# xbpeng/DeepMimic

Hardware: NVIDIA H100
Metric: env-steps/sec (30 Hz policy steps; humanoid3d_spinkick, 4096 envs/GPU) (higher is better)
Workload: dtype f32

## Files before the change

deepmimic_b200/csrc/kernels/dm_step.cu:

```cuda
#include "dm_model.cuh"
#include <type_traits>

namespace dmk {

namespace {

template <int W>
struct Tl {
    static __device__ __forceinline__ float shfl(float v, int src) { return __shfl_sync(0xffffffffu, v, src, W); }
    static __device__ __forceinline__ int shfli(int v, int src) { return __shfl_sync(0xffffffffu, v, src, W); }
    static __device__ __forceinline__ V3 shfl3(V3 v, int src) { return mk3(shfl(v.x, src), shfl(v.y, src), shfl(v.z, src)); }
    static __device__ __forceinline__ S6 shfl6(S6 v, int src) { return mks(shfl3(v.a, src), shfl3(v.l, src)); }
};
__device__ __forceinline__ void ld12(const float* p, float* o) {
    const float4 a = reinterpret_cast<const float4*>(p)[0], b = reinterpret_cast<const float4*>(p)[1], c_ = reinterpret_cast<const float4*>(p)[2];
    o[0] = a.x; o[1] = a.y; o[2] = a.z; o[3] = a.w; o[4] = b.x; o[5] = b.y; o[6] = b.z; o[7] = b.w; o[8] = c_.x; o[9] = c_.y; o[10] = c_.z; o[11] = c_.w;
}
__device__ __forceinline__ void st12(float* p, const float* o) {
    reinterpret_cast<float4*>(p)[0] = make_float4(o[0], o[1], o[2], o[3]); reinterpret_cast<float4*>(p)[1] = make_float4(o[4], o[5], o[6], o[7]);
    reinterpret_cast<float4*>(p)[2] = make_float4(o[8], o[9], o[10], o[11]);
}
__device__ __forceinline__ float rcp_fast(float x) { float r; asm("rcp.approx.ftz.f32 %0, %1;" : "=f"(r) : "f"(x)); return r; }
__device__ __forceinline__ int wmax(int v) {
#pragma unroll
// ... 14 lines not shown
        t[0 + j] = s[0] * R.m[j] + s[1] * R.m[3 + j] + s[2] * R.m[6 + j];
        t[3 + j] = s[1] * R.m[j] + s[3] * R.m[3 + j] + s[4] * R.m[6 + j];
        t[6 + j] = s[2] * R.m[j] + s[4] * R.m[3 + j] + s[5] * R.m[6 + j];
    }
    o[0] = R.m[0] * t[0] + R.m[3] * t[3] + R.m[6] * t[6];
    o[1] = R.m[0] * t[1] + R.m[3] * t[4] + R.m[6] * t[7];
    o[2] = R.m[0] * t[2] + R.m[3] * t[5] + R.m[6] * t[8];
    o[3] = R.m[1] * t[1] + R.m[4] * t[4] + R.m[7] * t[7];
    o[4] = R.m[1] * t[2] + R.m[4] * t[5] + R.m[7] * t[8];
    o[5] = R.m[2] * t[2] + R.m[5] * t[5] + R.m[8] * t[8];
}
__device__ __forceinline__ float normalize_angle3(float t) {
    float n = fmodf(t, 6.283185307179586f);
    if (n > 3.14159265358979f) n -= 6.283185307179586f;
    else if (n < -3.14159265358979f) n += 6.283185307179586f;
    return n;
}
__device__ __forceinline__ V3 quat_rotvec3(Q4 q) {
    float s = sqrtf(q.x * q.x + q.y * q.y + q.z * q.z);
    if (!(s > 0.000001f)) return mk3(0.f, 0.f, 0.f);
    float th = normalize_angle3(2.0f * atan2f(s, q.w));
    float k = th / s;
    return mk3(q.x * k, q.y * k, q.z * k);
}
__device__ __forceinline__ Q4 quat_integrate3(V3 omega, Q4 quat, bool base_body, float dt) {
    V3 angvel = base_body ? omega : qrot(quat, omega);
    float fAngle = sqrtf(dot(angvel, angvel));
    const float kThr = 0.5f * 1.57079632679489661923f;
    if (fAngle * dt > kThr) fAngle = kThr / dt;
    V3 axis;
    if (fAngle < 0.001f) axis = angvel * (0.5f * dt - (dt * dt * dt) * 0.020833333333f * fAngle * fAngle);
    else axis = angvel * (__sinf(0.5f * fAngle * dt) / fAngle);
    float cw = __cosf(fAngle * dt * 0.5f);
    Q4 r = base_body ? qmul(quat, mkq(-axis.x, -axis.y, -axis.z, cw)) : qmul(mkq(axis.x, axis.y, axis.z, cw), quat);
    float n = rsqrtf(r.x * r.x + r.y * r.y + r.z * r.z + r.w * r.w);
    return mkq(r.x * n, r.y * n, r.z * n, r.w * n);
}

enum LkSlot { kLC = 0 , kLM = 3,
              kLD = 4 , kLThr = 7,
              kLWd = 8 , kLInt = 14 , kLInt2 = 15 ,
              kLWb = 16 , kLFlg = 22 , kLTree = 23 ,
              kLAx = 24 , kLTl = 27,
              kLZr = 28 ,
              kLHe = 32 , kLKp = 35,
              kLKd = 36, kLLo = 37, kLHi = 38, kLChild = 39 ,
              kLDc = 40 , kLMc = 43 ,
              kLDyn = 44 , kLDChild = 45 ,
              kLkFloats = 48 };
__device__ __forceinline__ float4 ld4(const float* p) { return *reinterpret_cast<const float4*>(p); }
enum HdrSlot { kHLayout = 0, kHLvc = 24, kHGrav = 32 , kHh = 35, kHScale = 36, kHMu = 37, kHFdt = 38, kHDmax = 39 , kHdrFloats = 40 };
__device__ __forceinline__ float* step_smem() { extern __shared__ __align__(16) float dm_step_sm[]; return dm_step_sm; }

}

int dm_step_layout(int nl, int n, int chain_len, int maxrows, int W, StepLayout* L) {
    const int maxpts = maxrows / 3;
    int o = 0;
    L->nl = nl; L->n = n; L->chain_len = chain_len; L->maxrows = maxrows; L->maxpts = maxpts;
    L->oU = o; o += nl * 24;
    L->oR = o; o += nl * 12;
    L->oA = o;
    const int world = nl * 24, tri = maxrows * (maxrows + 1) / 2;
    L->oW = o; L->oV = o + nl * 12;
    L->oPp = o + world; L->oQ = L->oPp + maxpts * 4;
    const int pre = world + maxpts * 4 + 4 * 8;
    o += (pre > tri ? pre : tri);
    o = (o + 3) & ~3;
    const int ys = dm_step_y_stride(W), scr = 28 * (nl - 1);
    L->oY = o; o += (chain_len * ys > scr) ? chain_len * ys : scr;
    L->oLam = o; o += maxrows; o += (o & 1); L->oRhs = o; o += maxrows; L->oInv = o; o += maxrows;
    L->oRl = o; o += maxrows;
    L->oPi = o; o += maxpts; L->oPr = o; o += maxpts;
    L->oG = o; o += 21 + 13 + 2;
    L->oZ = o; o += ((n + 3) / 4) * 4;
    L->env_floats = ((o + 15) / 32) * 32 + 16;
    L->hot_floats = kHdrFloats + ((nl * kLkFloats + (nl * nl + nl * chain_len + 3) / 4 + 3) / 4) * 4;
    return L->hot_floats * 4 + 0;
}
int dm_step_smem_bytes(const StepLayout& L, int tiles) { return (L.hot_floats + L.env_floats * tiles) * static_cast<int>(sizeof(float)); }

constexpr int kSubstepBarriers = 2;
constexpr int kPgsBlock = 2;
enum PgsSection { kSecLimit = 0, kSecNormal = 1, kSecFriction = 2 };
template <int W, int S, int ST, int B>
__device__ __forceinline__ void pgs_sweeps(const float* sA, float* sLam, const float2* sRI, int lane, int NL, int P, int NLmax, int Pmax, float mu) {
    using T = Tl<W>;
    float w[S];
#pragma unroll
    for (int s = 0; s < S; ++s) w[s] = 0.f;
    int tjs[S];
#pragma unroll
    for (int s = 0; s < S; ++s) { const int rid = lane + s * W; tjs[s] = rid * (rid + 1) / 2; }
    auto tri = [](int i) { return (i * (i + 1)) >> 1; };
    auto a_own = [&](int s, int i, int ti) -> float {
        if (ST > 0) return sA[i * ST + lane + s * W];
        const int rid = lane + s * W;
        return sA[(rid >= i) ? (tjs[s] + i) : (ti + rid)];
    };
    auto a_pair = [&](int i, int j, int ti, int tj_) -> float {
        if (ST > 0) return sA[i * ST + j];
        return sA[(i >= j) ? (ti + j) : (tj_ + i)];
    };
#pragma unroll 1
    for (int p = 0; p < Pmax; ++p) {
        const int i = NL + ((p < P) ? p : 0);
        const float l0 = (p < P) ? sLam[i] : 0.f;
#pragma unroll
        for (int s = 0; s < S; ++s) w[s] = fmaf(a_own(s, i, tri(i)), l0, w[s]);
    }
    bool writer[B];
#pragma unroll
    for (int k = 0; k < B; ++k) writer[k] = lane == k;
    auto block = [&](int pos0, int it, auto sec_tag) {
        constexpr int SEC = decltype(sec_tag)::value;
        int ik[B], tk[B]; bool vk[B];
        float tot = 0.f;
        float wk[B], rhs[B], inv[B], lam[B], lo[B], hi[B], ain[B * (B - 1) / 2 > 0 ? B * (B - 1) / 2 : 1], ao[S][B];
        if (SEC == kSecLimit) {
#pragma unroll
            for (int k = 0; k < B; ++k) { const int pos = pos0 + k; vk[k] = pos < NL; ik[k] = vk[k] ? ((it & 1) ? pos : NL - 1 - pos) : 0; }
        } else {
            const int i0 = ((SEC == kSecNormal) ? NL : NL + P) + pos0, cnt = (SEC == kSecNormal) ? P : 2 * P;
#pragma unroll
            for (int k = 0; k < B; ++k) { ik[k] = i0 + k; vk[k] = pos0 + k < cnt; }
        }
#pragma unroll
        for (int k = 0; k < B; ++k) tk[k] = (ST > 0) ? 0 : tri(ik[k]);
// ... 133 lines not shown
                        f.a.x -= ti * ub.z; f.a.y -= ti * ub.w; f.a.z -= ti * uc.x; f.l.x -= ti * uc.y; f.l.y -= ti * uc.z; f.l.z -= ti * uc.w;
                    }
                }
                if (nd >= 1) {
                    float t = qa.x * f.a.x + qa.y * f.a.y + qa.z * f.a.z;
                    if (first && kind == 0) { t = lsign; rvel = lsign * sQ[24 + rid]; }
                    const float y = t * uf.y;
                    if (rv_) sY[dp0 * YS + rid] = y;
                    acc += y * y;
                    const float ti = t * ue.z;
                    f.a.x -= ti * ua.x; f.a.y -= ti * ua.y; f.a.z -= ti * ua.z; f.l.x -= ti * ua.w; f.l.y -= ti * ub.x; f.l.z -= ti * ub.y;
                }
                first = false;
                f = shift_f(f, mk3(qc.y, qc.z, qc.w));
                if (par < 0) break;
                cur = par;
            }
            {
                float x[6] = {f.a.x, f.a.y, f.a.z, f.l.x, f.l.y, f.l.z};
                int o = 0;
#pragma unroll
                for (int i = 0; i < 6; ++i) {
#pragma unroll
                    for (int k = 0; k < i; ++k) x[i] -= sG[o++] * x[k];
                    x[i] *= sG[15 + i];
                    if (rv_) sY[i * YS + rid] = x[i];
                    acc += x[i] * x[i];
                }
            }
            if (rv_) {
                const float inv = acc > 1.1920929e-7f ? 1.0f / acc : 0.f;
                float rhs, lam0 = 0.f;
                if (kind == 1) {
                    float perr = 0.f, verr = -rvel;
                    if (pdist > 0.f) verr -= pdist / h; else perr = -pdist * 0.2f / h;
                    rhs = perr * inv + verr * inv;
                    lam0 = sPi[p] * 0.85f;
                } else if (kind != 0) rhs = -rvel * inv;
                else {
                    float perr = 0.f, verr = -rvel;
                    const bool combine = lpen > -0.04f;
                    if (lpen > 0.f) verr = -lpen / h; else perr = -lpen * 0.2f / h;
                    rhs = combine ? (perr * inv + verr * inv) : (verr * inv);
                }
                sRI[rid] = make_float2(rhs, inv); sLam[rid] = lam0;
            }
        }
    }
    __syncwarp();
    SPROF(7);
    const int Pmax = (W == 32) ? P : wmax(P);
    const int NLmax = (W == 32) ? NL : wmax(NL);
    {
        constexpr int kSq2 = (W == 16) ? 22 : 36;
        const int region = max(nl * 24, MR * (MR + 1) / 2);
        const int mode = (nslots == 1) ? 0 : ((NRmax <= kSq2 && kSq2 * kSq2 + W <= region) ? 1 : 2);
        const int st = (mode == 0) ? W : kSq2;
        auto put = [&](int i, int j, float v) {
            if (mode != 2) { sA[i * st + j] = v; sA[j * st + i] = v; }
            else { const int hi_ = max(i, j), lo_ = min(i, j); sA[hi_ * (hi_ + 1) / 2 + lo_] = v; }
        };
#pragma unroll 1
        for (int j = 0; j < NLmax; ++j) {
            const bool jv = j < NL;
            const int bj = jv ? sRl[j] : 0;
#pragma unroll 1
            for (int i0 = 0; i0 < NRmax; i0 += W) {
                const int i = i0 + lane;
                const bool pv = jv && i < NR && i >= j;
                const int cd = pv ? CD[sRl[i] * nl + bj] : 0;
                const float* yi = sY + (pv ? i : 0); const float* yj = sY + (jv ? j : 0);
                float acc = 0.f;
#pragma unroll 1
                for (int k = 0; k < CL; k += 4, yi += 4 * YS, yj += 4 * YS) {
                    const float a0 = yi[0], a1 = yi[YS], a2 = yi[2 * YS], a3 = yi[3 * YS];
                    const float b0 = yj[0], b1 = yj[YS], b2 = yj[2 * YS], b3 = yj[3 * YS];
                    if (k < cd) acc += a0 * b0;
                    if (k + 1 < cd) acc += a1 * b1;
                    if (k + 2 < cd) acc += a2 * b2;
                    if (k + 3 < cd) acc += a3 * b3;
                }
                if (pv) put(i, j, acc);
            }
        }
        const int npp = P * (P + 1) / 2, nppmax = Pmax * (Pmax + 1) / 2;
#pragma unroll 1
        for (int q0 = 0; q0 < nppmax; q0 += W) {
            const int q = q0 + lane;
            const bool pv = q < npp;
            int pp = static_cast<int>((sqrtf(8.0f * static_cast<float>(q) + 1.0f) - 1.0f) * 0.5f);
            if (pp * (pp + 1) / 2 > q) --pp;
            if ((pp + 1) * (pp + 2) / 2 <= q) ++pp;
            const int pr = q - pp * (pp + 1) / 2;
            const int in_p = pv ? NL + pp : 0, it_p = pv ? NL + P + 2 * pp : 0, in_r = pv ? NL + pr : 0, it_r = pv ? NL + P + 2 * pr : 0;
            const int cd = pv ? CD[sRl[in_p] * nl + sRl[in_r]] : 0;
            const float* ypn = sY + in_p; const float* ypt = sY + it_p; const float* yrn = sY + in_r; const float* yrt = sY + it_r;
            float acc[3][3];
#pragma unroll
            for (int x = 0; x < 3; ++x)
#pragma unroll
                for (int y = 0; y < 3; ++y) acc[x][y] = 0.f;
#pragma unroll 1
            for (int k = 0; k < CL; k += 4, ypn += 4 * YS, ypt += 4 * YS, yrn += 4 * YS, yrt += 4 * YS) {
                float av[3][4], bv[3][4];
#pragma unroll
                for (int d = 0; d < 4; ++d) {
                    av[0][d] = ypn[d * YS]; av[1][d] = ypt[d * YS]; av[2][d] = ypt[d * YS + 1];
                    bv[0][d] = yrn[d * YS]; bv[1][d] = yrt[d * YS]; bv[2][d] = yrt[d * YS + 1];
                }
#pragma unroll
                for (int d = 0; d < 4; ++d)
                    if (k + d < cd) {
#pragma unroll
                        for (int x = 0; x < 3; ++x)
#pragma unroll
                            for (int y = 0; y < 3; ++y) acc[x][y] += av[x][d] * bv[y][d];
                    }
            }
            if (pv) {
                if (mode != 2) {
                    float* rp[3] = {sA + in_p * st, sA + it_p * st, sA + it_p * st + st};
                    float* rr[3] = {sA + in_r * st, sA + it_r * st, sA + it_r * st + st};
                    const int cp[3] = {in_p, it_p, it_p + 1}, cr[3] = {in_r, it_r, it_r + 1};
#pragma unroll
                    for (int x = 0; x < 3; ++x)
#pragma unroll
                        for (int y = 0; y < 3; ++y) { rp[x][cr[y]] = acc[x][y]; rr[y][cp[x]] = acc[x][y]; }
                } else {
#pragma unroll
                    for (int x = 0; x < 3; ++x)
#pragma unroll
                        for (int y = 0; y < 3; ++y) put(x == 0 ? in_p : it_p + x - 1, y == 0 ? in_r : it_r + y - 1, acc[x][y]);
                }
            }
        }
        __syncwarp();
        SPROF(8);
        if (mode == 0) pgs_sweeps<W, 1, W, kPgsBlock>(sA, sLam, sRI, lane, NL, P, NLmax, Pmax, mu);
        else if (mode == 1) pgs_sweeps<W, kSlots, kSq2, kPgsBlock>(sA, sLam, sRI, lane, NL, P, NLmax, Pmax, mu);
        else pgs_sweeps<W, kSlots, 0, kPgsBlock>(sA, sLam, sRI, lane, NL, P, NLmax, Pmax, mu);
    }
    SPROF(9);
#pragma unroll 1
    for (int p = lane; p < P; p += W) {
        if (alive) {
            const int ref = sPr[p];
            float* mpt = mani + (ref >> 2) * kManifoldFloats + (ref & 3) * 12;
            mpt[7] = sLam[NL + p]; mpt[8] = sLam[NL + P + 2 * p]; mpt[9] = sLam[NL + P + 2 * p + 1];
        }
    }
    {
        const int info = (lane < nl) ? lk_i(lane) : 0;
        const int nd = (info >> 16) & 0xff, dp0 = (info >> 24) & 0xff;
        const int d0 = (lane < nl) ? (lk_i2(lane) & 0xff) : 0;
        float z0 = 0.f, z1 = 0.f, z2 = 0.f, zb = 0.f;
        const int kb = (lane < 6) ? lane : 0;
        const bool mine = lane < nl && nd > 0;
        const int need = dp0 + nd - 1;
        const unsigned char* cdl = CD + lane;
#pragma unroll 2
        for (int i = 0; i < NRmax; ++i) {
            const int b = sRl[i];
            const float l = (i < NR) ? sLam[i] : 0.f;
            const float yb = sY[kb * YS + i], y0 = sY[dp0 * YS + i], y1 = sY[(dp0 + 1) * YS + i], y2 = sY[(dp0 + 2) * YS + i];
            const bool in = mine && cdl[b * nl] > need;
            zb = fmaf(yb, l, zb);
            if (in) { z0 = fmaf(y0, l, z0); if (nd == 3) { z1 = fmaf(y1, l, z1); z2 = fmaf(y2, l, z2); } }
        }
        if (lane < 6) sZ[lane] = zb;
        if (lane < nl && nd >= 1) sZ[d0] = z0;
        if (lane < nl && nd == 3) { sZ[d0 + 1] = z1; sZ[d0 + 2] = z2; }
    }
    __syncwarp();
}


struct Ctx {
    float* E;
    const int* LYS;
    const float* LK;
    int lane, li;
    int plane, level, ndof, jtype, maxlevel;
    bool act;
};
__device__ __forceinline__ const StepLayout& lay_of(const Ctx& c) { return *reinterpret_cast<const StepLayout*>(c.LYS); }
template <int W>
__device__ __forceinline__ Ctx make_ctx() {
    Ctx c;
    float* sm = step_smem();
    c.LYS = reinterpret_cast<const int*>(sm + kHLayout); c.LK = sm + kHdrFloats;
    const StepLayout& LY = *reinterpret_cast<const StepLayout*>(c.LYS);
    const int tile = threadIdx.x / W;
    c.lane = threadIdx.x % W;
// ... 23 lines not shown
template <int W>
__device__ __noinline__ void kin_pass(float4 jp, float4 jv) {
    const Ctx c = make_ctx<W>();
    using T = Tl<W>;
    const StepLayout& LY = lay_of(c);
    float* sS = c.E + LY.oR; float* sW = c.E + LY.oW; float* sV = c.E + LY.oV; const float* sB = c.E + LY.oG + 21;
    const float* LKo = c.LK + c.li * kLkFloats;
    const float4 ax4 = ld4(LKo + kLAx), zr4 = ld4(LKo + kLZr), c4 = ld4(LKo + kLC);
    const V3 axis = mk3(ax4.x, ax4.y, ax4.z);
    const Q4 zrot = mkq(zr4.x, zr4.y, zr4.z, zr4.w);
    const V3 cvec = mk3(c4.x, c4.y, c4.z);
    Q4 cached;
    if (c.jtype == kJSpherical) cached = qmul(mkq(jp.x, jp.y, jp.z, -jp.w), zrot);
    else if (c.jtype == kJRevolute) {
        float s, co;
        __sincosf(-0.5f * jp.x, &s, &co);
        cached = qmul(mkq(axis.x * s, axis.y * s, axis.z * s, co), zrot);
    } else cached = zrot;
    const M3 R = qmat(cached);
    V3 jw = mk3(0, 0, 0);
    if (c.jtype == kJSpherical) jw = mk3(jv.x, jv.y, jv.z); else if (c.jtype == kJRevolute) jw = jv.x * axis;
    M3 Rwl; V3 Pw, cw; S6 vel;
    if (c.lane == 0) {
        const M3 Rwb = qmat(mkq(sB[3], sB[4], sB[5], sB[6]));
        const V3 bo = mk3(sB[7], sB[8], sB[9]);
        Rwl = mul(R, Rwb); cw = mulT(Rwb, cvec); Pw = mk3(sB[0], sB[1], sB[2]) + cw;
        vel = mks(bo + mulT(Rwl, jw), mk3(sB[10], sB[11], sB[12]) + cross(bo, cw));
    }
#pragma unroll 1
    for (int lv = 1; lv <= c.maxlevel; ++lv) {
        M3 pR; V3 pp; S6 pv;
#pragma unroll
        for (int k = 0; k < 9; ++k) pR.m[k] = T::shfl(Rwl.m[k], c.plane);
        pp = T::shfl3(Pw, c.plane);
        pv = T::shfl6(vel, c.plane);
        if (c.level == lv) {
            Rwl = mul(R, pR); cw = mulT(pR, cvec); Pw = pp + cw;
            vel = mks(pv.a + mulT(Rwl, jw), pv.l + cross(pv.a, cw));
        }
    }
    if (c.act) {
        const float4 d4 = ld4(LKo + kLD);
        const V3 dw = mulT(Rwl, mk3(d4.x, d4.y, d4.z));
        V3 S0 = mk3(Rwl.m[0], Rwl.m[1], Rwl.m[2]);
        if (c.jtype != kJSpherical) S0 = mulT(Rwl, axis);
        const float wr[12] = {Rwl.m[0], Rwl.m[1], Rwl.m[2], Rwl.m[3], Rwl.m[4], Rwl.m[5], Rwl.m[6], Rwl.m[7], Rwl.m[8], Pw.x, Pw.y, Pw.z};
        const float qr[12] = {S0.x, S0.y, S0.z, Rwl.m[3], Rwl.m[4], Rwl.m[5], Rwl.m[6], Rwl.m[7], Rwl.m[8], cw.x, cw.y, cw.z};
        const float vr[12] = {vel.a.x, vel.a.y, vel.a.z, vel.l.x, vel.l.y, vel.l.z, dw.x, dw.y, dw.z, 0.f, 0.f, 0.f};
        st12(sW + c.lane * 12, wr); st12(sS + c.lane * 12, qr); st12(sV + c.lane * 12, vr);
    }
    __syncwarp();
}

template <int W>
__device__ __noinline__ int collide(float* mani, int alive, int mcnt) {
    const Ctx c = make_ctx<W>();
    const float scale = step_smem()[kHScale];
    using T = Tl<W>;
    const StepLayout& LY = lay_of(c);
    const float* sW = c.E + LY.oW; const float* sV = c.E + LY.oV;
    float* sPp = c.E + LY.oPp; float* sPi = c.E + LY.oPi; int* sPr = reinterpret_cast<int*>(c.E + LY.oPr);
    const float* LKo = c.LK + c.li * kLkFloats;
    const int shape = reinterpret_cast<const int*>(LKo)[kLFlg] & 0xff;
    int cnt = 0;
    float mp[48];
    M3 Rwl;
    float wrec[12], vrec[12];
    ld12(sW + c.li * 12, wrec); ld12(sV + c.li * 12, vrec);
#pragma unroll
    for (int k = 0; k < 9; ++k) Rwl.m[k] = wrec[k];
    const float thr = LKo[kLThr];
    const float4 he4 = ld4(LKo + kLHe);
    const V3 he = mk3(he4.x, he4.y, he4.z);
    const V3 pos = mk3(wrec[9] + vrec[6], wrec[10] + vrec[7], wrec[11] + vrec[8]);
    V3 dl = mul(Rwl, mk3(0.f, -1.f, 0.f));
    V3 vtx;
    if (shape == kSBox) vtx = mk3(dl.x >= 0 ? he.x : -he.x, dl.y >= 0 ? he.y : -he.y, dl.z >= 0 ? he.z : -he.z);
    else {
        V3 sup = mk3(0, 0, 0);
        if (shape == kSCapsule) sup = mk3(0.f, (dl.y >= 0.f) ? he.y : -he.y, 0.f);
        float inv = rsqrtf(dot(dl, dl));
        vtx = sup + (he.x * inv) * dl;
    }
    const V3 vw = pos + mulT(Rwl, vtx);
    const float dist = vw.y;
    const bool need = c.act && alive && (mcnt > 0 || dist < thr);
    {
        const float4* mg = reinterpret_cast<const float4*>(mani + c.li * kManifoldFloats);
#pragma unroll
        for (int k = 0; k < 12; ++k) { float4 v = need ? mg[k] : make_float4(0.f, 0.f, 0.f, 0.f); mp[4 * k] = v.x; mp[4 * k + 1] = v.y; mp[4 * k + 2] = v.z; mp[4 * k + 3] = v.w; }
    }
#pragma unroll
    for (int k = 0; k < 4; ++k) if (mp[k * 12] != 0.f && cnt == k) cnt = k + 1;
    if (c.act && dist < thr) {
        float best = thr * thr; int nearest = -1;
#pragma unroll
        for (int k = 0; k < 4; ++k) if (k < cnt) {
            float dx = mp[k * 12 + 1] - vtx.x, dy = mp[k * 12 + 2] - vtx.y, dz = mp[k * 12 + 3] - vtx.z, dd = dx * dx + dy * dy + dz * dz;
            if (dd < best) { best = dd; nearest = k; }
        }
        int idx = nearest;
        float k7 = 0, k8 = 0, k9 = 0, k11 = 0;
        if (nearest >= 0) {
#pragma unroll
            for (int k = 0; k < 4; ++k) if (k == nearest) { k7 = mp[k * 12 + 7]; k8 = mp[k * 12 + 8]; k9 = mp[k * 12 + 9]; k11 = mp[k * 12 + 11]; }
        } else if (cnt < 4) { idx = cnt; cnt++; }
        else {
            int mpi = -1; float mpen = dist;
#pragma unroll
            for (int k = 0; k < 4; ++k) if (mp[k * 12 + 10] < mpen) { mpi = k; mpen = mp[k * 12 + 10]; }
            auto Pt = [&](int k) { return mk3(mp[k * 12 + 1], mp[k * 12 + 2], mp[k * 12 + 3]); };
            auto area = [&](V3 a, V3 b) { V3 x = cross(a, b); return dot(x, x); };
            float res[4] = {0, 0, 0, 0};
            if (mpi != 0) res[0] = area(vtx - Pt(1), Pt(3) - Pt(2));
            if (mpi != 1) res[1] = area(vtx - Pt(0), Pt(3) - Pt(2));
            if (mpi != 2) res[2] = area(vtx - Pt(0), Pt(3) - Pt(1));
            if (mpi != 3) res[3] = area(vtx - Pt(0), Pt(2) - Pt(1));
            idx = 0; float bv = fabsf(res[0]);
#pragma unroll
            for (int k = 1; k < 4; ++k) if (fabsf(res[k]) > bv) { bv = fabsf(res[k]); idx = k; }
        }
#pragma unroll
        for (int k = 0; k < 4; ++k) if (k == idx) {
            float* q = mp + k * 12;
            q[0] = 1.f; q[1] = vtx.x; q[2] = vtx.y; q[3] = vtx.z; q[4] = vw.x; q[5] = 0.f; q[6] = vw.z; q[7] = k7; q[8] = k8; q[9] = k9; q[10] = dist; q[11] = k11;
        }
    }
#pragma unroll
    for (int k = 3; k >= 0; --k) if (k < cnt) {
        V3 pa = pos + mulT(Rwl, mk3(mp[k * 12 + 1], mp[k * 12 + 2], mp[k * 12 + 3]));
        mp[k * 12 + 10] = pa.y - mp[k * 12 + 5];
        mp[k * 12 + 11] += 1.f;
    }
#pragma unroll
    for (int k = 3; k >= 0; --k) if (k < cnt) {
        V3 pa = pos + mulT(Rwl, mk3(mp[k * 12 + 1], mp[k * 12 + 2], mp[k * 12 + 3]));
        bool rm = !(mp[k * 12 + 10] <= thr);
        if (!rm) {
            float dx = mp[k * 12 + 4] - pa.x, dy = mp[k * 12 + 5] - (pa.y - mp[k * 12 + 10]), dz = mp[k * 12 + 6] - pa.z;
            rm = (dx * dx + dy * dy + dz * dz) > thr * thr;
        }
        if (rm) {
            const int last = cnt - 1;
#pragma unroll
            for (int l2 = 0; l2 < 4; ++l2) if (l2 == last) {
                if (k != l2) for (int j = 0; j < 12; ++j) mp[k * 12 + j] = mp[l2 * 12 + j];
                mp[l2 * 12] = 0.f;
            }
            cnt--;
        }
    }
    if (!c.act || !alive) cnt = 0;
    int tol = 0;
#pragma unroll
    for (int k = 0; k < 4; ++k) if (k < cnt && mp[k * 12 + 10] <= 0.001f * scale) tol = 1;
    if (need) {
        float4* mo = reinterpret_cast<float4*>(mani + c.li * kManifoldFloats);
#pragma unroll
        for (int k = 0; k < 12; ++k) mo[k] = make_float4(mp[4 * k], mp[4 * k + 1], mp[4 * k + 2], mp[4 * k + 3]);
    }
    int incl = cnt, over = 0;
#pragma unroll
    for (int o = 1; o < W; o <<= 1) { int t = __shfl_up_sync(0xffffffffu, incl, o, W); if (c.lane >= o) incl += t; }
    const int base = incl - cnt;
#pragma unroll
    for (int k = 0; k < 4; ++k) if (k < cnt) {
        const int p = base + k;
        if (p < LY.maxpts) {
            V3 pa = pos + mulT(Rwl, mk3(mp[k * 12 + 1], mp[k * 12 + 2], mp[k * 12 + 3]));
            sPp[p * 4] = pa.x; sPp[p * 4 + 1] = pa.y; sPp[p * 4 + 2] = pa.z; sPp[p * 4 + 3] = mp[k * 12 + 10];
            sPi[p] = mp[k * 12 + 7];
            sPr[p] = c.lane * 4 + k;
        } else over = 1;
    }
    const int P = min(T::shfli(incl, W - 1), LY.maxpts);
    __syncwarp();
    return P | (tol << 8) | (over << 9) | (cnt << 10);
}

template <int W>
__device__ __noinline__ float3 aba_solve(float g0, float g1, float g2, float kdt, int bullet, float jvx, float jvy, float jvz) {
    const Ctx c = make_ctx<W>();
    const float gx = step_smem()[kHGrav], gy = step_smem()[kHGrav + 1], gz = step_smem()[kHGrav + 2], h = step_smem()[kHh];
    using T = Tl<W>;
    const StepLayout& LY = lay_of(c);
    float* sU = c.E + LY.oU; const float* sS = c.E + LY.oR; const float* sW = c.E + LY.oW; float* sV = c.E + LY.oV; float* sG = c.E + LY.oG; float* sB = sG + 21;
    const float* LKo = c.LK + c.li * kLkFloats;
    const int dyn = c.act ? reinterpret_cast<const int*>(LKo)[kLDyn] : (100 << 8);
    const int dpar = dyn & 0xff, dlev = static_cast<int>(static_cast<signed char>((dyn >> 8) & 0xff)), byp = (dyn >> 16) & 0xff, dnch = (dyn >> 24) & 0xff;
    const int dchild = reinterpret_cast<const int*>(LKo)[kLDChild];
    const int dmax = reinterpret_cast<const int*>(step_smem())[kHDmax];
    const bool isroot = c.lane == 0;
    const float4 dc4 = ld4(LKo + kLDc);
    const float mass = c.act ? dc4.w : 0.f;
    float q[12];
    ld12(sS + c.li * 12, q);
    const V3 S0 = mk3(q[0], q[1], q[2]), S1 = mk3(q[3], q[4], q[5]), S2 = mk3(q[6], q[7], q[8]), cwk = mk3(q[9], q[10], q[11]);
    V3 cw = cwk;
    if (byp != 0xff) { const float* qb = sS + byp * 12; cw = cw + mk3(qb[9], qb[10], qb[11]); }
    if (isroot) cw = mk3(0, 0, 0);
    float vv[8];
    {
        const float4 a = reinterpret_cast<const float4*>(sV + c.li * 12)[0], b = reinterpret_cast<const float4*>(sV + c.li * 12)[1];
        vv[0] = a.x; vv[1] = a.y; vv[2] = a.z; vv[3] = a.w; vv[4] = b.x; vv[5] = b.y;
    }
    const S6 velk = mks(mk3(vv[0], vv[1], vv[2]), mk3(vv[3], vv[4], vv[5]));
    S6 vel = velk;
    if (isroot) vel = mks(mk3(sB[7], sB[8], sB[9]), mk3(sB[10], sB[11], sB[12]));
    V3 jww = mk3(0, 0, 0);
    if (c.jtype == kJSpherical) jww = jvx * S0 + jvy * S1 + jvz * S2; else if (c.jtype == kJRevolute) jww = jvx * S0;
    S6 ab;
    {
        const S6 cj = mks(cross(vel.a, jww), cross(vel.l, jww));
        if (isroot) {
            const V3 bo = vel.a, bv = vel.l;
            V3 wxv;
            if (bullet) wxv = cross(bo, bv);
            else {
                const M3 Rwb = qmat(mkq(sB[3], sB[4], sB[5], sB[6]));
                wxv = mulT(Rwb, cross(bo, mul(Rwb, bv)));
            }
            ab = mks(mk3(0, 0, 0), mk3(-gx, -gy, -gz) - wxv);
        }
#pragma unroll 1
        for (int lv = 0; lv <= dmax; ++lv) {
            S6 pa = T::shfl6(ab, dpar);
            if (dlev == lv) ab = shift_m(pa, cw) + cj;
        }
    }
    Art IA; S6 pA;
// ... 472 lines not shown
        }
        PROF(1);
        if (stage == total_stages) break;
        if (__syncthreads_and(!alive)) break;
        PROF(2);
        if (__ballot_sync(0xffffffffu, alive) == 0u) {
            if ((stage % stages_per_upd) != 0)
                for (int k = 0; k < kSubstepBarriers; ++k) __syncthreads();
            continue;
        }
        const int ph = stage % stages_per_upd;
        if (ph == 0) {
            int cb = 0;
            if constexpr (TASK) {
                if (__ballot_sync(0xffffffffu, alive && need_action) != 0u) {
                    const V3 com = tile_com<W>(E + LY.oW + li * 12, sV + li * 12, act ? LKo[kLM] : 0.f, 1.0f / (M.total_mass * scale));
                    if (lane == 0 && alive && need_action) { tk[kKPrevCom] = com.x; tk[kKPrevCom + 1] = com.y; tk[kKPrevCom + 2] = com.z; }
                }
            }
            if (lane == 0 && alive) {
                const double timer = tm[kTTimer] + dt;
                double kin_time = tm[kTKin];
                double dur_ = M.motion_dur;
                if constexpr (TASK) dur_ = st.ctab->info[st.clip[env]].dur;
                const double dur = dur_;
                double p0 = kin_time / dur; p0 -= floor(p0);
                kin_time += dt;
                double p1 = kin_time / dur; p1 -= floor(p1);
                if constexpr (TASK) {
                    const ClipInfo& ci = st.ctab->info[st.clip[env]];
                    if (ci.loop && p1 < p0 && M.sync_root_pos) {
                        const double simq[4] = {static_cast<double>(sB[3]), static_cast<double>(sB[4]), static_cast<double>(sB[5]), static_cast<double>(sB[6])};
                        kin_wrap_sync(frame_times + ci.frame_off, frames + static_cast<size_t>(ci.frame_off) * M.pose_dim, M.pose_dim, ci.num_frames, ci.cycle_delta, dur, kin_time,
                                      tm + kTOrigin, tm + kTOriginRot, static_cast<double>(sB[0]) / M.scale, static_cast<double>(sB[2]) / M.scale, simq, true, false);
                    }
                } else if (M.loop_motion && p1 < p0 && (M.sync_root_pos || M.sync_root_rot)) {
                    const double simq[4] = {static_cast<double>(sB[3]), static_cast<double>(sB[4]), static_cast<double>(sB[5]), static_cast<double>(sB[6])};
                    kin_wrap_sync(frame_times, frames, M.pose_dim, M.num_frames, M.cycle_delta, dur, kin_time, tm + kTOrigin, tm + kTOriginRot,
                                  static_cast<double>(sB[0]) / M.scale, static_cast<double>(sB[2]) / M.scale, simq, M.sync_root_pos != 0, M.sync_root_rot != 0);
                }
                const double ctrl_time = tm[kTCtrl] + dt;
                if (need_action) tm[kTPrevAct] = ctrl_time;
                tm[kTTimer] = timer; tm[kTKin] = kin_time; tm[kTCtrl] = ctrl_time;
                {
                    const double cur = ctrl_time + tm[kTInitOff], pad = 0.001 * dt, T_ = M.query_dt;
                    int c0 = static_cast<int>(floor((cur + pad) / T_)), c1 = static_cast<int>(floor((cur + pad - dt) / T_));
                    cb = (c0 != c1) ? 1 : 0;
                }
                if (timer >= tm[kTTimerMax]) cb |= 2;
                if (M.end_at_clip_end && kin_time >= dur) cb |= 4;
            }
            cbits = T::shfli(cb, 0);
            need_action = 0;
            PROF(3);
            const float4 tg = reinterpret_cast<const float4*>(sim + 16 + 8 * nl)[li];
            float e0 = 0, e1 = 0, e2 = 0;
            if (jtype == kJSpherical) {
                Q4 q = mkq(jp.x, jp.y, jp.z, jp.w);
                Q4 dq = qmul(q, mkq(jv.x, jv.y, jv.z, 0.f));
                Q4 qi = qnormalize(mkq(q.x + 0.5f * fdt * dq.x, q.y + 0.5f * fdt * dq.y, q.z + 0.5f * fdt * dq.z, q.w + 0.5f * fdt * dq.w));
                V3 e = quat_rotvec3(qmul(qconj(qi), mkq(tg.x, tg.y, tg.z, tg.w)));
                e0 = e.x; e1 = e.y; e2 = e.z;
            } else if (jtype == kJRevolute) {
                e0 = tg.x - (normalize_angle3(jp.x) + fdt * jv.x);
            }
            const float kp = LKo[kLKp], kd = LKo[kLKd];
            const float pe0 = kp * e0, pe1 = kp * e1, pe2 = kp * e2;
            const float3 qdd = aba_solve<W>(pe0 - kd * jv.x, pe1 - kd * jv.y, pe2 - kd * jv.z, fdt * kd, 0, jv.x, jv.y, jv.z);
            float t0 = 0, t1 = 0, t2 = 0;
            if (ndof >= 1) t0 = pe0 + kd * (-jv.x - fdt * qdd.x);
            if (ndof == 3) { t1 = pe1 + kd * (-jv.y - fdt * qdd.y); t2 = pe2 + kd * (-jv.z - fdt * qdd.z); }
            const float mag = sqrtf(t0 * t0 + t1 * t1 + t2 * t2), tlim = LKo[kLTl];
            if (mag > tlim) { float s = tlim / mag; t0 *= s; t1 *= s; t2 *= s; }
            tau0 = t0; tau1 = t1; tau2 = t2;
            PROF(4);
            continue;
        }
        int P;
        {
            const int r = collide<W>(mani, alive ? 1 : 0, mcnt);
            P = r & 0xff; in_contact_tol = ((r >> 8) & 1) != 0; if ((r >> 9) & 1) f_over = 1; mcnt = (r >> 10) & 7;
        }
        PROF(3);
        {
            const float3 qdd = aba_solve<W>(tau0, tau1, tau2, 0.f, 1, jv.x, jv.y, jv.z);
            bool hit = false;
            if (ndof >= 1) { const float v = jv.x + h * qdd.x; jv.x = cl100(v); hit |= fabsf(v) > 100.f; }
            if (ndof == 3) { const float v1 = jv.y + h * qdd.y, v2 = jv.z + h * qdd.z; jv.y = cl100(v1); jv.z = cl100(v2); hit |= fabsf(v1) > 100.f || fabsf(v2) > 100.f; }
            if (lane == 0) for (int k = 0; k < 6; ++k) hit |= fabsf(sB[7 + k]) >= 100.f;
            const unsigned hb = __ballot_sync(0xffffffffu, hit);
            if (hb != 0u) {
                const unsigned hseg = (W == 32) ? hb : ((hb >> (threadIdx.x & 16)) & 0xffffu);
                vel_pass<W>(jv.x, jv.y, jv.z, hseg != 0u);
            }
        }
        PROF(ph == 1 ? 16 : 17);
        __syncthreads();
        PROF(2);
        int lim_dir = 0; float lim_pen = 0.f;
        if (act && has_limit && alive) {
            float p0 = jp.x - LKo[kLLo], p1 = LKo[kLHi] - jp.x;
            if (!(p0 > 0.f)) { lim_dir = 1; lim_pen = p0; }
            else if (!(p1 > 0.f)) { lim_dir = -1; lim_pen = p1; }
        }
        const unsigned lbal = __ballot_sync(0xffffffffu, lim_dir != 0);
        const unsigned lseg = (W == 32) ? lbal : ((lbal >> (threadIdx.x & 16)) & 0xffffu);
        int NL = __popc(lseg);
        const unsigned anyrow = __ballot_sync(0xffffffffu, NL + P > 0);
        last_nr = 0;
        if (anyrow != 0) {
            {
                const int lidx = __popc(lseg & ((1u << lane) - 1u));
                if (NL > 8) { NL = 8; f_over = 1; }
                if (lim_dir != 0 && lidx < 8) { sQ[lidx] = __int_as_float(lane); sQ[8 + lidx] = (lim_dir == -1) ? -1.f : 1.f; sQ[16 + lidx] = lim_pen; sQ[24 + lidx] = jv.x; }
            }
            if (NL + 3 * P > LY.maxrows) { P = (LY.maxrows - NL) / 3; f_over = 1; }
            const int NR = NL + 3 * P;
            last_nr = NR;
            __syncwarp();
            PROF(5);
#ifdef DM_PROFILE
            { const int nrm = wmax(NR); if ((threadIdx.x & 31) == 0) { PRF[13] += nrm; PRF[14] += 1; if (nrm > W) PRF[15] += 1; } }
#endif
            solve_rows<W>(NL, P, mani, alive ? 1 : 0, PRFP);
            PROF(10);
            const float3 dq = dv_pass<W>();
            if (NR > 0) {
                if (ndof >= 1) jv.x = cl100(jv.x + dq.x);
                if (ndof == 3) { jv.y = cl100(jv.y + dq.y); jv.z = cl100(jv.z + dq.z); }
            }
            PROF(11);
        }
        __syncthreads();
        PROF(2);
        if (lane == 0) {
            sB[0] += h * sB[10]; sB[1] += h * sB[11]; sB[2] += h * sB[12];
            const Q4 q = quat_integrate3(mk3(sB[7], sB[8], sB[9]), mkq(sB[3], sB[4], sB[5], sB[6]), true, h);
            sB[3] = q.x; sB[4] = q.y; sB[5] = q.z; sB[6] = q.w;
        }
        if (jtype == kJRevolute) jp.x += h * jv.x;
        else if (jtype == kJSpherical) { Q4 q = quat_integrate3(mk3(jv.x, jv.y, jv.z), mkq(jp.x, jp.y, jp.z, jp.w), false, h); jp = make_float4(q.x, q.y, q.z, q.w); }
        __syncwarp();
        need_kin = true;
        if (ph == sim_substeps) pending_flags = true;
        PROF(12);
    }
#ifdef DM_PROFILE
    __syncwarp();
    if ((threadIdx.x & 31) == 0 && st.prof) { unsigned int* o = st.prof + (blockIdx.x * (blockDim.x / 32) + threadIdx.x / 32) * kProfCounters; for (int k = 0; k < kProfCounters; ++k) o[k] = PRF[k]; }
#endif
}

const StepKernel kStepKernels[2][2] = {{dm_step_kernel<16, false>, dm_step_kernel<16, true>}, {dm_step_kernel<32, false>, dm_step_kernel<32, true>}};

constexpr int kEnvOrderItems = 4;
__global__ void __launch_bounds__(kEnvOrderThreads) dm_env_order_kernel(const int* __restrict__ load, int n_padded, int tiles, int W, int* __restrict__ order) {
    constexpr int kWarps = kEnvOrderThreads / 32, kCells = kEnvOrderItems * kWarps, kChunk = kEnvOrderItems * kEnvOrderThreads;
    constexpr int kParts = kEnvOrderThreads / kLoadBuckets, kPer = kCells / kParts;
    static_assert(kParts <= 32 && 32 % kParts == 0 && kCells % kParts == 0, "the scan of a bucket's cells runs inside one warp");
    __shared__ int base[kLoadBuckets];
    __shared__ int cnt[kLoadBuckets][kCells + 1];
    const int t = threadIdx.x, warp = t / 32, lane = t % 32;
    const unsigned lt = (1u << lane) - 1u;
    int b[kEnvOrderItems];
    auto load_chunk = [&](int c0) {
#pragma unroll
        for (int i = 0; i < kEnvOrderItems; ++i) { const int e = c0 + i * kEnvOrderThreads + t; b[i] = (e < n_padded) ? env_load_bucket(load[e]) : kLoadBuckets; }
    };
    auto count = [&](int bk) {
        const unsigned peers = __match_any_sync(0xffffffffu, bk);
        if (bk < kLoadBuckets && (peers & lt) == 0) atomicAdd(&base[bk], __popc(peers));
    };
    load_chunk(0);
    if (t < kLoadBuckets) base[t] = 0;
    __syncthreads();
// ... 48 lines not shown
```

Before: 2.513 million.

## Enlarge W=16 square PGS matrix region and alias scratch arrays into it

For 16-wide tiles, the square (non-packed) PGS matrix stride grows from 22 to 24. The layout now reserves at least a 24x24 region, so the square mode is always chosen when the row count fits, rather than falling back to packed triangular indexing. To pay for the larger region, the Pi and Z scratch arrays are aliased into the same region for W=16, which shrinks the per-env footprint elsewhere. This risks lifetime conflicts between the aliased buffers and the matrix, and it changes shared-memory size and therefore occupancy. Profiling counters and a compile-time switch to force packed mode are also added.

After: 2.579 million (median of 6 runs). +2.6%, better.

```diff
diff --git a/deepmimic_b200/csrc/kernels/dm_step.cu b/deepmimic_b200/csrc/kernels/dm_step.cu
--- a/deepmimic_b200/csrc/kernels/dm_step.cu
+++ b/deepmimic_b200/csrc/kernels/dm_step.cu
@@ -90,6 +90,8 @@
 enum HdrSlot { kHLayout = 0, kHLvc = 24, kHGrav = 32 , kHh = 35, kHScale = 36, kHMu = 37, kHFdt = 38, kHDmax = 39 , kHdrFloats = 40 };
 __device__ __forceinline__ float* step_smem() { extern __shared__ __align__(16) float dm_step_sm[]; return dm_step_sm; }
 
+__host__ __device__ constexpr int pgs_sq2(int W) { return W == 16 ? 24 : 36; }
+
 }
 
 int dm_step_layout(int nl, int n, int chain_len, int maxrows, int W, StepLayout* L) {
@@ -102,16 +104,22 @@
     const int world = nl * 24, tri = maxrows * (maxrows + 1) / 2;
     L->oW = o; L->oV = o + nl * 12;
     L->oPp = o + world; L->oQ = L->oPp + maxpts * 4;
-    const int pre = world + maxpts * 4 + 4 * 8;
-    o += (pre > tri ? pre : tri);
+    int pre = world + maxpts * 4 + 4 * 8, region = tri;
+    if (W == 16) {
+        L->oPi = o + pre; pre += maxpts;
+        L->oZ = o;
+        if (pgs_sq2(W) * pgs_sq2(W) > region) region = pgs_sq2(W) * pgs_sq2(W);
+    }
+    o += (pre > region ? pre : region);
     o = (o + 3) & ~3;
     const int ys = dm_step_y_stride(W), scr = 28 * (nl - 1);
     L->oY = o; o += (chain_len * ys > scr) ? chain_len * ys : scr;
     L->oLam = o; o += maxrows; o += (o & 1); L->oRhs = o; o += maxrows; L->oInv = o; o += maxrows;
     L->oRl = o; o += maxrows;
-    L->oPi = o; o += maxpts; L->oPr = o; o += maxpts;
+    if (W != 16) { L->oPi = o; o += maxpts; }
+    L->oPr = o; o += maxpts;
     L->oG = o; o += 21 + 13 + 2;
-    L->oZ = o; o += ((n + 3) / 4) * 4;
+    if (W != 16) { L->oZ = o; o += ((n + 3) / 4) * 4; }
     L->env_floats = ((o + 15) / 32) * 32 + 16;
     L->hot_floats = kHdrFloats + ((nl * kLkFloats + (nl * nl + nl * chain_len + 3) / 4 + 3) / 4) * 4;
     return L->hot_floats * 4 + 0;
@@ -351,9 +359,13 @@
     const int Pmax = (W == 32) ? P : wmax(P);
     const int NLmax = (W == 32) ? NL : wmax(NL);
     {
-        constexpr int kSq2 = (W == 16) ? 22 : 36;
+        constexpr int kSq2 = pgs_sq2(W);
         const int region = max(nl * 24, MR * (MR + 1) / 2);
-        const int mode = (nslots == 1) ? 0 : ((NRmax <= kSq2 && kSq2 * kSq2 + W <= region) ? 1 : 2);
+#ifdef DM_PGS_PACKED
+        const int mode = (nslots == 1) ? 0 : 2;
+#else
+        const int mode = (nslots == 1) ? 0 : ((NRmax <= kSq2 && (W == 16 || kSq2 * kSq2 + W <= region)) ? 1 : 2);
+#endif
         const int st = (mode == 0) ? W : kSq2;
         auto put = [&](int i, int j, float v) {
             if (mode != 2) { sA[i * st + j] = v; sA[j * st + i] = v; }
@@ -438,6 +450,9 @@
         if (mode == 0) pgs_sweeps<W, 1, W, kPgsBlock>(sA, sLam, sRI, lane, NL, P, NLmax, Pmax, mu);
         else if (mode == 1) pgs_sweeps<W, kSlots, kSq2, kPgsBlock>(sA, sLam, sRI, lane, NL, P, NLmax, Pmax, mu);
         else pgs_sweeps<W, kSlots, 0, kPgsBlock>(sA, sLam, sRI, lane, NL, P, NLmax, Pmax, mu);
+#ifdef DM_PROFILE
+        if (mode != 0 && (threadIdx.x & 31) == 0) prf[6] += static_cast<unsigned int>(clock64()) - pt;
+#endif
     }
     SPROF(9);
 #pragma unroll 1
@@ -1337,7 +1352,10 @@
             __syncwarp();
             PROF(5);
 #ifdef DM_PROFILE
-            { const int nrm = wmax(NR); if ((threadIdx.x & 31) == 0) { PRF[13] += nrm; PRF[14] += 1; if (nrm > W) PRF[15] += 1; } }
+            {
+                const int nrm = wmax(NR);
+                if ((threadIdx.x & 31) == 0) { PRF[13] += nrm; PRF[14] += 1; if (nrm > W) PRF[15] += (nrm > pgs_sq2(W)) ? 65536u : 1u; }
+            }
 #endif
             solve_rows<W>(NL, P, mani, alive ? 1 : 0, PRFP);
             PROF(10);
```

## Process contact manifolds with four lanes per link instead of one

Applied to the files above, without the earlier changes.

Contact manifold update in collide is restructured so each link needing collision work is handled by a quad of lanes, one per cached contact point, processed in compacted passes via ballots. This removes the 48-float per-thread manifold array, which is large in registers or local memory, and the serial per-point loops. The cost is extra shuffles, ballots and a pass loop, plus explicit rounding intrinsics to keep results matching. A profiling marker index also changes.

New measurement: 2.531 million before, 2.577 million after, median of 6. 1.8% higher.

```diff
diff --git a/deepmimic_b200/csrc/kernels/dm_step.cu b/deepmimic_b200/csrc/kernels/dm_step.cu
--- a/deepmimic_b200/csrc/kernels/dm_step.cu
+++ b/deepmimic_b200/csrc/kernels/dm_step.cu
@@ -567,6 +567,31 @@
     __syncwarp();
 }
 
+__device__ __forceinline__ V3 link_point(const M3& R, V3 pos, V3 p) {
+    return mk3(__fadd_rn(pos.x, __fmaf_rn(R.m[6], p.z, __fmaf_rn(R.m[0], p.x, __fmul_rn(R.m[3], p.y)))),
+               __fadd_rn(pos.y, __fmaf_rn(R.m[7], p.z, __fmaf_rn(R.m[1], p.x, __fmul_rn(R.m[4], p.y)))),
+               __fadd_rn(pos.z, __fmaf_rn(R.m[8], p.z, __fmaf_rn(R.m[2], p.x, __fmul_rn(R.m[5], p.y)))));
+}
+
+template <int W>
+__device__ __forceinline__ int sort_cached_points(V3 own, float own_dist, V3 p, float dist) {
+    const int s = threadIdx.x & 3, q0 = (threadIdx.x % W) & ~3;
+    auto qshfl = [&](float x, int k) { return Tl<W>::shfl(x, q0 + k); };
+    int mpi = -1; float mpen = dist;
+#pragma unroll
+    for (int k = 0; k < 4; ++k) { const float pen = qshfl(own_dist, k); if (pen < mpen) { mpi = k; mpen = pen; } }
+    auto pt = [&](int k) { return mk3(qshfl(own.x, k), qshfl(own.y, k), qshfl(own.z, k)); };
+    const V3 pa = pt(s == 0 ? 1 : 0), pb = pt(s == 3 ? 2 : 3), pc = pt(s <= 1 ? 2 : 1);
+    const float ax = p.x - pa.x, ay = p.y - pa.y, az = p.z - pa.z;
+    const float bx = pb.x - pc.x, by = pb.y - pc.y, bz = pb.z - pc.z;
+    const float cx = __fmaf_rn(ay, bz, -__fmul_rn(az, by)), cy = __fmaf_rn(az, bx, -__fmul_rn(ax, bz)), cz = __fmaf_rn(ax, by, -__fmul_rn(ay, bx));
+    const float area = (mpi != s) ? __fmaf_rn(cz, cz, __fmaf_rn(cx, cx, __fmul_rn(cy, cy))) : 0.f;
+    int idx = 0; float bv = fabsf(qshfl(area, 0));
+#pragma unroll
+    for (int k = 1; k < 4; ++k) { const float a = fabsf(qshfl(area, k)); if (a > bv) { bv = a; idx = k; } }
+    return idx;
+}
+
 template <int W>
 __device__ __noinline__ int collide(float* mani, int alive, int mcnt) {
     const Ctx c = make_ctx<W>();
@@ -577,8 +602,6 @@
     float* sPp = c.E + LY.oPp; float* sPi = c.E + LY.oPi; int* sPr = reinterpret_cast<int*>(c.E + LY.oPr);
     const float* LKo = c.LK + c.li * kLkFloats;
     const int shape = reinterpret_cast<const int*>(LKo)[kLFlg] & 0xff;
-    int cnt = 0;
-    float mp[48];
     M3 Rwl;
     float wrec[12], vrec[12];
     ld12(sW + c.li * 12, wrec); ld12(sV + c.li * 12, vrec);
@@ -597,100 +620,119 @@
         float inv = rsqrtf(dot(dl, dl));
         vtx = sup + (he.x * inv) * dl;
     }
-    const V3 vw = pos + mulT(Rwl, vtx);
+    const V3 vw = link_point(Rwl, pos, vtx);
     const float dist = vw.y;
     const bool need = c.act && alive && (mcnt > 0 || dist < thr);
-    {
-        const float4* mg = reinterpret_cast<const float4*>(mani + c.li * kManifoldFloats);
-#pragma unroll
-        for (int k = 0; k < 12; ++k) { float4 v = need ? mg[k] : make_float4(0.f, 0.f, 0.f, 0.f); mp[4 * k] = v.x; mp[4 * k + 1] = v.y; mp[4 * k + 2] = v.z; mp[4 * k + 3] = v.w; }
-    }
-#pragma unroll
-    for (int k = 0; k < 4; ++k) if (mp[k * 12] != 0.f && cnt == k) cnt = k + 1;
-    if (c.act && dist < thr) {
-        float best = thr * thr; int nearest = -1;
-#pragma unroll
-        for (int k = 0; k < 4; ++k) if (k < cnt) {
-            float dx = mp[k * 12 + 1] - vtx.x, dy = mp[k * 12 + 2] - vtx.y, dz = mp[k * 12 + 3] - vtx.z, dd = dx * dx + dy * dy + dz * dz;
-            if (dd < best) { best = dd; nearest = k; }
-        }
+    constexpr int Q = W / 4;
+    const unsigned nb = __ballot_sync(0xffffffffu, need);
+    const unsigned tneed = (W == 32) ? nb : ((nb >> (threadIdx.x & 16)) & 0xffffu);
+    const int passes = (((W == 32) ? __popc(tneed) : max(__popc(nb & 0xffffu), __popc(nb >> 16))) + Q - 1) / Q;
+    const int rank = __popc(tneed & ((1u << c.lane) - 1u));
+    const int s = c.lane & 3, qlane = c.lane & ~3;
+    const unsigned qshift = threadIdx.x & 28;
+    int res = 0;
+    int carry = 0;
+    unsigned rest = tneed;
+#pragma unroll 1
+    for (int t = 0; t < passes; ++t) {
+        unsigned m = rest;
+#pragma unroll
+        for (int k = 1; k < Q; ++k) if (k <= (c.lane >> 2)) m &= m - 1u;
+        const bool qv = m != 0u;
+        const int L = qv ? __ffs(m) - 1 : 0;
+#pragma unroll
+        for (int k = 0; k < Q; ++k) rest &= rest - 1u;
+        const V3 lvtx = T::shfl3(vtx, L);
+        const float lvwx = T::shfl(vw.x, L), lvwz = T::shfl(vw.z, L), ldist = T::shfl(dist, L);
+        const float lthr = c.LK[L * kLkFloats + kLThr], thr2 = __fmul_rn(lthr, lthr);
+        M3 R;
+        V3 lpos;
+        {
+            float w_[12];
+            ld12(sW + L * 12, w_);
+            const float* v_ = sV + L * 12;
+#pragma unroll
+            for (int k = 0; k < 9; ++k) R.m[k] = w_[k];
+            lpos = mk3(w_[9] + v_[6], w_[10] + v_[7], w_[11] + v_[8]);
+        }
+        float* const mq = mani + L * kManifoldFloats + s * 12;
+        float q[12];
+        if (qv) ld12(mq, q);
+        else {
+#pragma unroll
+            for (int k = 0; k < 12; ++k) q[k] = 0.f;
+        }
+        int cnt = __ffs(~((__ballot_sync(0xffffffffu, q[0] != 0.f) >> qshift) & 0xfu)) - 1;
+        const bool ins = qv && ldist < lthr;
+        float dd[4];
+        {
+            const float dx = q[1] - lvtx.x, dy = q[2] - lvtx.y, dz = q[3] - lvtx.z, d2 = __fmaf_rn(dz, dz, __fmaf_rn(dx, dx, __fmul_rn(dy, dy)));
+#pragma unroll
+            for (int k = 0; k < 4; ++k) dd[k] = T::shfl(d2, qlane + k);
+        }
+        float best = thr2; int nearest = -1;
+#pragma unroll
+        for (int k = 0; k < 4; ++k) if (k < cnt && dd[k] < best) { best = dd[k]; nearest = k; }
         int idx = nearest;
-        float k7 = 0, k8 = 0, k9 = 0, k11 = 0;
-        if (nearest >= 0) {
-#pragma unroll
-            for (int k = 0; k < 4; ++k) if (k == nearest) { k7 = mp[k * 12 + 7]; k8 = mp[k * 12 + 8]; k9 = mp[k * 12 + 9]; k11 = mp[k * 12 + 11]; }
-        } else if (cnt < 4) { idx = cnt; cnt++; }
-        else {
-            int mpi = -1; float mpen = dist;
-#pragma unroll
-            for (int k = 0; k < 4; ++k) if (mp[k * 12 + 10] < mpen) { mpi = k; mpen = mp[k * 12 + 10]; }
-            auto Pt = [&](int k) { return mk3(mp[k * 12 + 1], mp[k * 12 + 2], mp[k * 12 + 3]); };
-            auto area = [&](V3 a, V3 b) { V3 x = cross(a, b); return dot(x, x); };
-            float res[4] = {0, 0, 0, 0};
-            if (mpi != 0) res[0] = area(vtx - Pt(1), Pt(3) - Pt(2));
-            if (mpi != 1) res[1] = area(vtx - Pt(0), Pt(3) - Pt(2));
-            if (mpi != 2) res[2] = area(vtx - Pt(0), Pt(3) - Pt(1));
-            if (mpi != 3) res[3] = area(vtx - Pt(0), Pt(2) - Pt(1));
-            idx = 0; float bv = fabsf(res[0]);
-#pragma unroll
-            for (int k = 1; k < 4; ++k) if (fabsf(res[k]) > bv) { bv = fabsf(res[k]); idx = k; }
-        }
-#pragma unroll
-        for (int k = 0; k < 4; ++k) if (k == idx) {
-            float* q = mp + k * 12;
-            q[0] = 1.f; q[1] = vtx.x; q[2] = vtx.y; q[3] = vtx.z; q[4] = vw.x; q[5] = 0.f; q[6] = vw.z; q[7] = k7; q[8] = k8; q[9] = k9; q[10] = dist; q[11] = k11;
-        }
-    }
-#pragma unroll
-    for (int k = 3; k >= 0; --k) if (k < cnt) {
-        V3 pa = pos + mulT(Rwl, mk3(mp[k * 12 + 1], mp[k * 12 + 2], mp[k * 12 + 3]));
-        mp[k * 12 + 10] = pa.y - mp[k * 12 + 5];
-        mp[k * 12 + 11] += 1.f;
-    }
-#pragma unroll
-    for (int k = 3; k >= 0; --k) if (k < cnt) {
-        V3 pa = pos + mulT(Rwl, mk3(mp[k * 12 + 1], mp[k * 12 + 2], mp[k * 12 + 3]));
-        bool rm = !(mp[k * 12 + 10] <= thr);
-        if (!rm) {
-            float dx = mp[k * 12 + 4] - pa.x, dy = mp[k * 12 + 5] - (pa.y - mp[k * 12 + 10]), dz = mp[k * 12 + 6] - pa.z;
-            rm = (dx * dx + dy * dy + dz * dz) > thr * thr;
-        }
-        if (rm) {
-            const int last = cnt - 1;
-#pragma unroll
-            for (int l2 = 0; l2 < 4; ++l2) if (l2 == last) {
-                if (k != l2) for (int j = 0; j < 12; ++j) mp[k * 12 + j] = mp[l2 * 12 + j];
-                mp[l2 * 12] = 0.f;
-            }
-            cnt--;
-        }
-    }
-    if (!c.act || !alive) cnt = 0;
-    int tol = 0;
-#pragma unroll
-    for (int k = 0; k < 4; ++k) if (k < cnt && mp[k * 12 + 10] <= 0.001f * scale) tol = 1;
-    if (need) {
-        float4* mo = reinterpret_cast<float4*>(mani + c.li * kManifoldFloats);
-#pragma unroll
-        for (int k = 0; k < 12; ++k) mo[k] = make_float4(mp[4 * k], mp[4 * k + 1], mp[4 * k + 2], mp[4 * k + 3]);
-    }
-    int incl = cnt, over = 0;
-#pragma unroll
-    for (int o = 1; o < W; o <<= 1) { int t = __shfl_up_sync(0xffffffffu, incl, o, W); if (c.lane >= o) incl += t; }
-    const int base = incl - cnt;
-#pragma unroll
-    for (int k = 0; k < 4; ++k) if (k < cnt) {
-        const int p = base + k;
-        if (p < LY.maxpts) {
-            V3 pa = pos + mulT(Rwl, mk3(mp[k * 12 + 1], mp[k * 12 + 2], mp[k * 12 + 3]));
-            sPp[p * 4] = pa.x; sPp[p * 4 + 1] = pa.y; sPp[p * 4 + 2] = pa.z; sPp[p * 4 + 3] = mp[k * 12 + 10];
-            sPi[p] = mp[k * 12 + 7];
-            sPr[p] = c.lane * 4 + k;
-        } else over = 1;
-    }
-    const int P = min(T::shfli(incl, W - 1), LY.maxpts);
+        const bool sorts = ins && nearest < 0 && cnt == 4;
+        if (__any_sync(0xffffffffu, sorts)) { const int k = sort_cached_points<W>(mk3(q[1], q[2], q[3]), q[10], lvtx, ldist); if (sorts) idx = k; }
+        if (ins && nearest < 0 && cnt < 4) { idx = cnt; cnt++; }
+        if (ins && s == idx) {
+            if (nearest < 0) { q[7] = 0.f; q[8] = 0.f; q[9] = 0.f; q[11] = 0.f; }
+            q[0] = 1.f; q[1] = lvtx.x; q[2] = lvtx.y; q[3] = lvtx.z; q[4] = lvwx; q[5] = 0.f; q[6] = lvwz; q[10] = ldist;
+        }
+        bool rm = false;
+        V3 pa = mk3(0.f, 0.f, 0.f);
+        if (s < cnt) {
+            pa = link_point(R, lpos, mk3(q[1], q[2], q[3]));
+            q[10] = __fsub_rn(pa.y, q[5]);
+            q[11] = __fadd_rn(q[11], 1.f);
+            rm = !(q[10] <= lthr);
+            if (!rm) {
+                const float dx = q[4] - pa.x, dy = q[5] - (pa.y - q[10]), dz = q[6] - pa.z;
+                rm = __fmaf_rn(dz, dz, __fmaf_rn(dx, dx, __fmul_rn(dy, dy))) > thr2;
+            }
+        }
+        const unsigned rball = __ballot_sync(0xffffffffu, rm);
+        if (rball != 0u) {
+            const unsigned rq = (rball >> qshift) & 0xfu;
+            unsigned src = 0xe4u, zero = 0u;
+#pragma unroll
+            for (int k = 3; k >= 0; --k) if ((rq >> k) & 1u) {
+                const int last = cnt - 1;
+                const unsigned from = (src >> (2 * last)) & 3u;
+                src = (src & ~(3u << (2 * k))) | (from << (2 * k));
+                zero |= 1u << last;
+                cnt--;
+            }
+            const int from = qlane + static_cast<int>((src >> (2 * s)) & 3u);
+#pragma unroll
+            for (int k = 0; k < 12; ++k) q[k] = T::shfl(q[k], from);
+            pa = T::shfl3(pa, from);
+            if ((zero >> s) & 1u) q[0] = 0.f;
+        }
+        if (!qv) cnt = 0;
+        if (qv) st12(mq, q);
+        const unsigned tile_bits = (W == 32) ? 0xffffffffu : (0xffffu << (threadIdx.x & 16));
+        const unsigned vt = (__ballot_sync(0xffffffffu, s < cnt) & tile_bits) >> (threadIdx.x & (32 - W));
+        const unsigned tt = (__ballot_sync(0xffffffffu, s < cnt && q[10] <= __fmul_rn(0.001f, scale)) & tile_bits) >> (threadIdx.x & (32 - W));
+        const int base = carry + __popc(vt & ((1u << qlane) - 1u));
+        if (s < cnt && base + s < LY.maxpts) {
+            const int p = base + s;
+            reinterpret_cast<float4*>(sPp)[p] = make_float4(pa.x, pa.y, pa.z, q[10]);
+            sPi[p] = q[7];
+            sPr[p] = L * 4 + s;
+        }
+        if (need && rank / Q == t) {
+            const int sh = 4 * (rank - t * Q);
+            const int lcnt = __popc((vt >> sh) & 0xfu), lbase = carry + __popc(vt & ((1u << sh) - 1u));
+            res = lcnt | (((tt >> sh) & 0xfu) != 0u ? 8 : 0) | ((lcnt > 0 && lbase + lcnt > LY.maxpts) ? 16 : 0);
+        }
+        carry += __popc(vt);
+    }
+    const int P = min(carry, LY.maxpts);
     __syncwarp();
-    return P | (tol << 8) | (over << 9) | (cnt << 10);
+    return P | (((res >> 3) & 1) << 8) | (((res >> 4) & 1) << 9) | ((res & 7) << 10);
 }
 
 template <int W>
@@ -1269,7 +1311,7 @@
             }
             cbits = T::shfli(cb, 0);
             need_action = 0;
-            PROF(3);
+            PROF(6);
             const float4 tg = reinterpret_cast<const float4*>(sim + 16 + 8 * nl)[li];
             float e0 = 0, e1 = 0, e2 = 0;
             if (jtype == kJSpherical) {
```
